# PASSIONLab/ELBA

Hardware: AMD Instinct MI355X
Metric: overlap nnz/sec (A·Aᵀ SpGEMM, SharedSeeds semiring, after Prune(numshared<=1)) (higher is better)
Workload: dtype u32

## Files before the change

### elba_amd/csrc/capi.hip

```cpp
#include "common.hpp"
#include "ov_plan.hpp"
#include <new>

using namespace elba;

struct elba_ctx {
    Ctx c;
};

namespace {

template <class F>
int guarded(elba_ctx *ctx, F &&f)
{
    if (!ctx) return ELBA_ERR_INVALID_ARG;
    try {
        ELBA_HIP(hipSetDevice(ctx->c.device));
        f(ctx->c);
        return ELBA_OK;
    } catch (const Error &e) {
        ctx->c.last_error = e.msg;
        return e.code;
    } catch (const std::bad_alloc &) {
        ctx->c.last_error = "host allocation failed";
// ... 753 lines not shown
        if (has(c.v, P_COUNTS)) { c.pre_ready = false; c.pre_consumed = true; }
    });
}

int elba_get_stat(elba_ctx *ctx, const char *name, int64_t *value)
{
    return guarded(ctx, [&](Ctx &c) {
        ELBA_REQUIRE(name && value, ELBA_ERR_INVALID_ARG, "get_stat: null name or value");
        if (!strcmp(name, "overlap_mirror_placed")) *value = c.ov_mir_placed;
        else if (!strcmp(name, "overlap_slab_q16")) *value = (int64_t)c.ov_slab_q16_used;
        else if (!strcmp(name, "kmer_path")) *value = c.kmer_path;
        else if (!strcmp(name, "kmer_passes")) *value = c.kmer_passes;
        else if (!strcmp(name, "kmer_crowded_buckets")) *value = c.kmer_crowded;
        else if (!strcmp(name, "kmer_crowded_small")) *value = c.kmer_crowded_small;
        else if (!strcmp(name, "kmer_largest_pass")) *value = c.kmer_largest_pass;
        else if (!strcmp(name, "kmer_peak_bytes")) *value = c.kmer_peak_bytes;
        else if (!strcmp(name, "kmer_buckets")) *value = c.kmer_buckets;
        else if (!strcmp(name, "overlap_passes")) *value = c.ov_passes;
        else if (!strcmp(name, "overlap_spec")) *value = c.ov_spec;
        else if (!strcmp(name, "overlap_forwarded")) *value = c.ov_forwarded;
        else if (!strncmp(name, "overlap_tier_limit_", 19) && name[19] >= '0' && name[19] < '0' + NUM_LDS_TIERS && !name[20]) *value = c.ov_tier_limit[name[19] - '0'];
        else if (!strncmp(name, "overlap_tier_queued_", 20) && name[20] >= '0' && name[20] < '0' + NUM_TIERS && !name[21]) *value = c.ov_tier_queued[name[20] - '0'];
        else if (!strncmp(name, "overlap_tier_done_", 18) && name[18] >= '0' && name[18] < '0' + NUM_TIERS && !name[19]) *value = c.ov_tier_done[name[18] - '0'];
        else if (!strcmp(name, "overlap_sort_rows_bucket")) *value = c.ov_sort_rows[0];
        else if (!strcmp(name, "overlap_sort_rows_huge")) *value = c.ov_sort_rows[1];
        else if (!strcmp(name, "overlap_family")) *value = c.ov_family;
        else if (!strcmp(name, "overlap_pay16")) *value = c.ov_pay16;
        else if (!strcmp(name, "overlap_rec16")) *value = c.ov_rec16_used;
        else if (!strcmp(name, "matrix_col_stride")) *value = has(c.v, P_A) && c.use_ell ? (int64_t)c.s_stride : 0;
        else if (!strcmp(name, "matrix_fbits")) *value = has(c.v, P_A) ? (int64_t)c.fbits : 0;
// ... 170 lines not shown
```

### elba_amd/csrc/common.hpp

```cpp
#pragma once
#include <hip/hip_runtime.h>
#include <cstdint>
#include <cstdio>
#include <cstdlib>
#include <cstring>
#include <mutex>
#include <string>
#include <vector>
#include "../../include/elba_amd.h"
#include "state.hpp"
#include "msd_plan.hpp"

namespace elba {

struct Error {
    int code;
    std::string msg;
};

#define ELBA_HIP(expr)                                                                                   \
    do {                                                                                                 \
        hipError_t e__ = (expr);                                                                         \
        if (e__ != hipSuccess) {                                                                         \
            throw ::elba::Error{e__ == hipErrorOutOfMemory ? ELBA_ERR_OUT_OF_MEMORY : ELBA_ERR_HIP,      \
// ... 159 lines not shown

    int64_t nreads = 0, first_global_id = 0, packed_bytes = 0;
    const uint8_t *d_packed = nullptr;
    const uint64_t *d_byte_off = nullptr;
    const uint32_t *d_len = nullptr;
    DevBuf own_packed, own_byte_off, own_len;
    uint32_t max_read_len = 0;
    std::vector<uint32_t> h_len;
    std::vector<uint64_t> h_byte_off;
    bool tx_index = false;
    DevBuf tx_recs, tx_name_pos, tx_name_len;
    std::vector<elba_fasta_record_t> tx_h_recs; std::vector<uint64_t> tx_h_name_pos; std::vector<uint32_t> tx_h_name_len;

    int triples_path = 0;
    int kmer_passes = 1;
    int64_t kmer_crowded = 0, kmer_crowded_small = 0, kmer_largest_pass = 0;
    int64_t kmer_peak_bytes = 0;
    int64_t kmer_buckets = 0;
    int kmer_path = 0;
    int64_t I = 0, ndistinct = 0;
    DevBuf inst_off;
    DevBuf rel_kmers;
    DevBuf rel_kmers_lo;
    DevBuf rel_kmers_lo2;
    DevBuf rel_counts;
    DevBuf csr_words;
    bool pre_pairs = false;
    bool pre_ready = false, pre_consumed = false, pre_words = false, pre_hints = false, pre_hints_done = false, pre_ell_done = false, pre_inline = false, pre_inline_pending = false ; int pre_rs = 0, pre_pbi = 0; int pre_nb = 0, pre_pb = 0; uint64_t pre_maxpos = 0;
    bool csr_hints = false, ov_hints_used = false, ov_rec16 = false;
    bool csr_inline = false;
// ... 215 lines not shown
```

### elba_amd/csrc/kmer.hip

```cpp
#include <memory>
#include "common.hpp"
#include "matrix.hpp"

namespace elba {

namespace {

#include "kmer_enum.hpp"

__device__ __forceinline__ uint64_t mix64(uint64_t k)
{
    k ^= k >> 33; k *= 0xff51afd7ed558ccdULL; k ^= k >> 33; k *= 0xc4ceb9fe1a85ec53ULL; k ^= k >> 33;
    return k;
}

__global__ void k_sort_columns(const uint32_t *colptr, uint64_t *csc, uint64_t *kid_keys, uint64_t N)
{
    const uint64_t k = (uint64_t)blockIdx.x * blockDim.x + threadIdx.x;
    if (k >= N) return;
    const uint32_t c0 = colptr[k], c1 = colptr[k + 1];
    for (uint32_t a = c0 + 1; a < c1; ++a) {
        const uint64_t v = csc[a];
        uint32_t b = a;
        while (b > c0 && csc[b - 1] > v) { csc[b] = csc[b - 1]; --b; }
// ... 485 lines not shown

    std::vector<uint64_t> off((size_t)M + 1);
    uint64_t I = 0;
    uint32_t maxlen = 0;
    for (int64_t r = 0; r < M; ++r) { const uint32_t l = c.h_len[(size_t)r]; off[(size_t)r] = I; if ((int64_t)l >= k) I += (uint64_t)l - k + 1; maxlen = l > maxlen ? l : maxlen; }
    off[(size_t)M] = I;
    c.max_read_len = maxlen;
    size_t free0 = 0;
    if (k > 31) { size_t total = 0; ELBA_HIP(hipMemGetInfo(&free0, &total)); }
    if (I >= 0xFFFFFFF0ull && k <= 31) {
        ELBA_REQUIRE(k >= 9, ELBA_ERR_UNSUPPORTED, "count_kmers: more than 2^32 k-mer instances on one GPU need k >= 9 (the sort of short k-mers holds 32-bit places)");
        ELBA_REQUIRE(!c.opt.kmer_no_msd, ELBA_ERR_UNSUPPORTED, "count_kmers: more than 2^32 k-mer instances on one GPU need the value partition (option kmer_no_msd is set)");
        ELBA_REQUIRE(k <= 17 || c.cfg.upper <= 255, ELBA_ERR_UNSUPPORTED, "count_kmers: more than 2^32 k-mer instances on one GPU need UPPER <= 255 for k > 17 (the sort holds 32-bit places)");
    }
    c.I = (int64_t)I; c.kmer_passes = 1; c.kmer_peak_bytes = 0;
    c.kmer_crowded = 0; c.kmer_crowded_small = 0; c.kmer_largest_pass = (int64_t)I; c.kmer_buckets = 0;
    c.inst_off.reserve((size_t)(M + 1) * 8);
    ELBA_HIP(hipMemcpyAsync(c.inst_off.p, off.data(), (size_t)(M + 1) * 8, hipMemcpyHostToDevice, s));

    if (k > 31) {
        const int words = k > 64 ? 3 : 2;
        if (count_long_kmers_in_passes(c, I, words, free0, st)) { done(c.v, EV_COUNT_KMERS); return; }
        DevBuf khi, klo, klo2, val, i0, i1, t0, t1, s2buf;
        for (DevBuf *b : {&khi, &klo, &val, &i0, &i1, &t0, &t1}) b->reserve((size_t)(I + 2) * 8);
        if (words == 3) { klo2.reserve((size_t)(I + 2) * 8); s2buf.reserve((size_t)(I + 2) * 8); }
        c.ws_a.reserve((size_t)(I + 2) * 8); c.ws_b.reserve((size_t)(I + 2) * 8); c.ws_c.reserve((size_t)(I + 2) * 8);
        c.ws_e.reserve((size_t)(I + 2) * 4); c.ws_f.reserve((size_t)(I + 2) * 8);
        c.t_total.start(s);
        c.t_a.start(s);
        EnumParams e = make_enum(c);
        const uint64_t nblocks = (I + EN_PER_BLOCK - 1) / EN_PER_BLOCK;
// ... 929 lines not shown
```

### elba_amd/csrc/kmer_msd.hip

```cpp
#include "common.hpp"
#include "matrix.hpp"
#include "msd_plan.hpp"
#include <algorithm>

namespace elba {

namespace {

#include "kmer_enum.hpp"

constexpr int MT_THREADS = ELBA_MT_THREADS, MT_ITEMS = ELBA_MT_ITEMS, MT_MAXBINS = 1 << MT_MAXBITS;
constexpr int BK_THREADS = 1024;
constexpr uint32_t EW = 2048;
constexpr uint32_t KW = EW / 2 + 1;
constexpr uint32_t EPAD = 256;
constexpr uint32_t BK_TAB = 16384, BK_ENT = BK_TAB + 2048 + 128 + 2 * (KW + 1);
static_assert(BK_ENT % 2 == 0, "staged entries are 8-byte words");
constexpr size_t BK_LDS_EMIT = (size_t)BK_ENT * 4 + (size_t)(EW + EPAD) * 10;
constexpr int KPT = 8;
static_assert(MT_ITEMS * 64 <= (1 << IB_SHIFT) && MT_TILE % 4096 == 0 && MT_TILE <= 65536, "a wavefront's share of a tile lies inside one block of the instance -> read table; run-start bitmap words per lane; 16-bit ranks");

struct MsdParams {
    int k2;
    int b1, b2;
// ... 206 lines not shown
            for (int u = 0; u < 8; ++u) x[u] = t + u < t1 ? hist[(size_t)(t + u) * nb2 + d] : 0u;
#pragma unroll
            for (int u = 0; u < 8; ++u) if (t + u < t1) hist[(size_t)(t + u) * nb2 + d] = x[u] + base;
        }
    }
    if (b == gridDim.x - 1 && d == 0) b2start[(size_t)gridDim.x * nb2] = (uint32_t)I;
}

#ifdef ELBA_SCATTER_CLOCK
__device__ unsigned long long g_sc_phase[2][2][12];
#define ELBA_SSTAMP(k) do { if (lane == 0 && w < 2) { const unsigned long long tn = __builtin_amdgcn_s_memtime(); sph[k] += tn - stp; stp = tn; } } while (0)
#else
#define ELBA_SSTAMP(k) do { } while (0)
#endif
__device__ __forceinline__ void lds_sync_fwd() { asm volatile("s_waitcnt lgkmcnt(0)\n\ts_barrier" ::: "memory"); }
template <bool ENUM, bool FILTER = false>
__global__ __launch_bounds__(MT_THREADS) void k_msd_scatter(EnumParams e, const BlockInfo *block_read, MsdParams m, const uint64_t *in, SegTiles sg, int shift, int bits,
                                                           const uint32_t *hist_scanned, uint64_t *out, uint32_t ntiles, uint32_t dlo, uint32_t dhi)
{
    __shared__ uint32_t kept_s;
    constexpr int WAVES = MT_THREADS / 64, DPT = MT_MAXBINS / MT_THREADS > 0 ? MT_MAXBINS / MT_THREADS : 1;
    __shared__ uint32_t lcnt[MT_MAXBINS], lstart[MT_MAXBINS], gbase[MT_MAXBINS], wsum[WAVES];
    __shared__ uint64_t lkey[MT_TILE];
    __shared__ unsigned long long hbits[MT_TILE / 64];
    __shared__ uint32_t hpre[MT_TILE / 64], delta[MT_MAXBINS];
    const uint32_t nbins = 1u << bits, dmask = nbins - 1u;
    if (!ENUM) ntiles = sg.tile0[sg.nb1];
    const int lane = threadIdx.x & 63, w = threadIdx.x >> 6;
    const unsigned long long lane_le = (2ull << lane) - 1ull;
#ifdef ELBA_SCATTER_CLOCK
    unsigned long long sph[12] = {0,0,0,0,0,0,0,0,0,0,0,0}, stp = __builtin_amdgcn_s_memtime();
#endif
    uint64_t key[MT_ITEMS];
    uint32_t dig2[MT_ITEMS / 2];
    uint32_t count = 0, ncount = 0; (void)ncount;
    auto digit = [&](int it) -> uint32_t { return (dig2[it >> 1] >> ((it & 1) * 16)) & 0xFFFFu; };
    auto set_digit = [&](int it, uint32_t d) { if (it & 1) dig2[it >> 1] |= d << 16; else dig2[it >> 1] = d; };
    auto fetch = [&](uint32_t t, uint32_t &cnt) {
        if (ENUM) {
            const uint64_t tbase = (uint64_t)t * MT_TILE, base = tbase + (uint64_t)w * (MT_ITEMS * 64);
            const uint64_t left = e.I - tbase;
            cnt = left < (uint64_t)MT_TILE ? (uint32_t)left : (uint32_t)MT_TILE;
            const uint64_t vmask = (1ull << (m.k2 - m.b1)) - 1;
#pragma unroll
            for (int it = 0; it < MT_ITEMS; ++it) key[it] = 0;
#pragma unroll
            for (int q = 0; q < MT_ITEMS / 2; ++q) dig2[q] = 0xFFFFFFFFu;
            enum_consecutive(e, block_read, base, [&](int it, uint64_t km, uint32_t r, uint32_t p) {
                const uint32_t dg = (uint32_t)(km >> (64 - m.b1));
                if (FILTER && (dg < dlo || dg >= dhi)) return;
                key[it] = (((km >> (64 - m.k2)) & vmask) << m.PB) | ((uint64_t)r << m.pbits) | p;
                dig2[it >> 1] = (it & 1) ? (dig2[it >> 1] & 0xFFFFu) | (dg << 16) : (dig2[it >> 1] & 0xFFFF0000u) | dg;
            });
        } else {
            uint32_t bucket, start;
            seg_tile(sg, t, bucket, start, cnt);
            const uint32_t wb = (uint32_t)w * (MT_ITEMS * 64);
#pragma unroll
            for (int it = 0; it < MT_ITEMS; ++it) {
                const uint32_t q = wb + (uint32_t)it * 64 + lane;
                key[it] = q < cnt ? in[start + q] : 0;
            }
        }
    };
    auto digits_of_loaded = [&](uint32_t cnt) {
        if (ENUM) return;
        const uint32_t wb = (uint32_t)w * (MT_ITEMS * 64);
#pragma unroll
        for (int it = 0; it < MT_ITEMS; ++it) {
            const uint32_t q = wb + (uint32_t)it * 64 + lane;
            set_digit(it, q < cnt ? (uint32_t)(key[it] >> shift) & dmask : 0xFFFFu);
        }
    };
#ifndef ELBA_SCATTER_ENUM_MODE
#define ELBA_SCATTER_ENUM_MODE 2
#endif
    constexpr bool PIPE = !ENUM || ELBA_SCATTER_ENUM_MODE != 0;
#ifndef ELBA_SCATTER_RR
    const uint32_t first_tile = (gridDim.x & 7u) ? blockIdx.x : (blockIdx.x & 7u) * (gridDim.x >> 3) + (blockIdx.x >> 3);
#else
    const uint32_t first_tile = blockIdx.x;
#endif
#ifndef ELBA_SCATTER_NO_PIPE
    if (PIPE && first_tile < ntiles) fetch(first_tile, count);
#endif
#ifndef ELBA_SCATTER_ONE_TILE
    for (uint32_t tile = first_tile; tile < ntiles; tile += gridDim.x) {
#else
    const uint32_t tile = blockIdx.x;
    if (tile < ntiles) {
#endif
    ELBA_SSTAMP(0);
// ... 21 lines not shown
    __syncthreads();
    ELBA_SSTAMP(3);
    {
        uint32_t tot[DPT], both = 0;
#pragma unroll
        for (int u = 0; u < DPT; ++u) { const uint32_t d = DPT * threadIdx.x + u; tot[u] = d < nbins ? lcnt[d] : 0u; both += tot[u]; }
        uint32_t inc = both;
#pragma unroll
        for (int s2 = 1; s2 < 64; s2 <<= 1) { const uint32_t o = __shfl_up(inc, s2, 64); if (lane >= s2) inc += o; }
        if (lane == 63) wsum[w] = inc;
        __syncthreads();
        uint32_t run = inc - both;
        for (int ww = 0; ww < w; ++ww) run += wsum[ww];
#pragma unroll
        for (int u = 0; u < DPT; ++u) { const uint32_t d = DPT * threadIdx.x + u; if (d < nbins) lstart[d] = run; run += tot[u]; }
        if (threadIdx.x == MT_THREADS - 1) kept_s = run;
#pragma unroll
        for (int u = 0; u < DPT; ++u) { const uint32_t d = threadIdx.x + u * MT_THREADS; if (d < nbins) gbase[d] = gb[u]; }
    }
    __syncthreads();
    ELBA_SSTAMP(4);
    if (ENUM && FILTER) count = kept_s;
#pragma unroll
    for (int it = 0; it < MT_ITEMS; ++it) {
        const uint32_t d = digit(it);
        if (d != 0xFFFFu) lkey[lstart[d] + rank[it]] = key[it];
    }
    ELBA_SSTAMP(5);
#ifdef ELBA_SCATTER_MEM_DIRECT
    if (!ENUM) {
#pragma unroll
        for (int u = 0; u < DPT; ++u) { const uint32_t d = DPT * threadIdx.x + u; if (d < nbins) delta[d] = gbase[d] - lstart[d]; }
        __syncthreads();
#pragma unroll
        for (int it = 0; it < MT_ITEMS; ++it) {
            const uint32_t t = (uint32_t)it * MT_THREADS + threadIdx.x;
            if (t < count) { const uint64_t kv = lkey[t]; out[delta[(uint32_t)(kv >> shift) & dmask] + t] = kv; }
        }
        __syncthreads();
#ifndef ELBA_SCATTER_ONE_TILE
        continue;
#else
        return;
#endif
    }
// ... 36 lines not shown
        const uint32_t t = (uint32_t)it * MT_THREADS + threadIdx.x;
        if (t < count) {
            const uint32_t run = hpre[t >> 6] + (uint32_t)__popcll(hbits[t >> 6] & ((2ull << (t & 63u)) - 1ull)) - 1u;
            out[delta[run] + t] = lkey[t];
        }
    }
#else
#if defined(ELBA_X_SCATTER) && ELBA_X_SCATTER == 1
    for (uint32_t t = threadIdx.x; t < count; t += MT_THREADS) out[(size_t)tile * MT_TILE + t] = lkey[t];
#elif defined(ELBA_X_SCATTER) && ELBA_X_SCATTER == 2
    for (uint32_t t = threadIdx.x; t < count; t += MT_THREADS) {
        const uint32_t run = hpre[t >> 6] + (uint32_t)__popcll(hbits[t >> 6] & lane_le) - 1u;
        if (delta[run] == 0xFFFFFFFEu) out[t] = lkey[t];
    }
#else
    if (ENUM) {
#pragma unroll 2
        for (uint32_t t = threadIdx.x; t < count; t += MT_THREADS) {
            const uint32_t run = hpre[t >> 6] + (uint32_t)__popcll(hbits[t >> 6] & lane_le) - 1u;
            out[delta[run] + t] = lkey[t];
        }
    } else
    for (uint32_t t = threadIdx.x; t < count; t += MT_THREADS) {
        const uint32_t run = hpre[t >> 6] + (uint32_t)__popcll(hbits[t >> 6] & lane_le) - 1u;
        out[delta[run] + t] = lkey[t];
    }
#endif
#endif
    };
#if !defined(ELBA_SCATTER_NO_PIPE) && !defined(ELBA_SCATTER_ONE_TILE)
    {
        const uint32_t nxt = tile + gridDim.x;
        const bool has = nxt < ntiles;
        if (!PIPE) writeout();
        else if (ENUM && ELBA_SCATTER_ENUM_MODE == 2 && (w & 1)) { writeout(); ELBA_SSTAMP(7); if (has) fetch(nxt, ncount); ELBA_SSTAMP(8); }
        else { if (has) fetch(nxt, ncount); ELBA_SSTAMP(8); writeout(); ELBA_SSTAMP(7); }
    }
#else
    writeout();
#endif
    lds_sync_fwd();
    ELBA_SSTAMP(9);
#ifndef ELBA_SCATTER_NO_PIPE
    if (PIPE) count = ncount;
#endif
    }
#ifdef ELBA_SCATTER_CLOCK
    if (lane == 0 && w < 2) for (int q = 0; q < 12; ++q) atomicAdd(&g_sc_phase[ENUM ? 1 : 0][w][q], sph[q]);
#endif
}

__device__ __forceinline__ void lds_sync() { asm volatile("s_waitcnt lgkmcnt(0)\n\ts_barrier" ::: "memory"); }

struct BucketStats { unsigned long long distinct, sumsq; unsigned int maxcol, ncrowded, nmid, nbig; };
struct BucketOut {
    uint64_t *rel_kmers; uint32_t *rel_counts, *colptr;
    uint64_t *csc, *csr_words, *kid_of_entry, *ell;
    uint32_t ell_stride;
    int nb, pb, rs, mb;
    uint32_t hints;
    uint32_t inl;
    unsigned long long *slot_cursor; uint32_t *slot_kid; uint32_t compact, slot_chunk;
    unsigned long long slot_cap;
    uint32_t *pair_key; uint64_t *pair_val;
// ... 1253 lines not shown

    void partition_triples()
    {
        const uint64_t I = pl.I;
        const uint32_t nb1 = pl.nb1, nb2 = pl.nb2, ntiles1 = pl.ntiles1, ntiles2 = pl.ntiles2;
        const SegTiles sg = seg();
        const uint32_t seg1[4] = {0u, (uint32_t)I, 0u, ntiles1};
        ELBA_HIP(hipMemcpyAsync(one_seg, seg1, sizeof(seg1), hipMemcpyHostToDevice, s));
        SegTiles sg1{one_seg, one_seg + 2, 1u};
        unsigned long long *badctr = reinterpret_cast<unsigned long long *>(one_seg + 4);
        ELBA_HIP(hipMemsetAsync(badctr, 0, 8, s));
        hipLaunchKernelGGL(k_pack_triple_msd, dim3((unsigned)((I + 255) / 256)), dim3(256), 0, s, tri->rows, tri->cols, tri->vals, I, tri->M, tri->N, m.pbits, m.PB, wb(), badctr);
        hipLaunchKernelGGL(k_msd_hist2, dim3(ntiles1), dim3(MT_THREADS), 0, s, (const uint64_t *)wb(), sg1, shift2() + m.b2, m.b1, hist());
        radix_column_scan(s, hist(), (int64_t)ntiles1, nb1, c.ws_scan);
        hipLaunchKernelGGL((k_tiles<MT_TILE, MT_MAXBINS>), dim3(1), dim3(MT_MAXBINS), 0, s, (const uint32_t *)hist(), nb1, I, b1start, tile0);
        hipLaunchKernelGGL((k_msd_scatter<false>), dim3(std::min<uint32_t>(ntiles1, sgrid())), dim3(MT_THREADS), 0, s, e, bi, m, (const uint64_t *)wb(), sg1, shift2() + m.b2, m.b1, (const uint32_t *)hist(), wa(), ntiles1, 0u, nb1);
        hipLaunchKernelGGL(k_msd_hist2, dim3(ntiles2), dim3(MT_THREADS), 0, s, (const uint64_t *)wa(), sg, shift2(), m.b2, hist());
        hipLaunchKernelGGL(k_msd_segscan, dim3(nb1), dim3(MT_MAXBINS), 0, s, hist(), sg, nb2, bt.b2start, I);
        hipLaunchKernelGGL((k_msd_scatter<false>), dim3(std::min<uint32_t>(ntiles2, sgrid())), dim3(MT_THREADS), 0, s, e, bi, m, (const uint64_t *)wa(), sg, shift2(), m.b2, (const uint32_t *)hist(), wb(), ntiles2, 0u, nb1);
        c.t_a.stop(s);
        c.t_b.start(s);
        ELBA_HIP(hipMemsetAsync(bt.gstat, 0, sizeof(BucketStats), s));
        hipLaunchKernelGGL(k_tri_stats, dim3((unsigned)std::min<uint32_t>(bt.nbuckets, (uint32_t)c.num_cus * 8u)), dim3(256), 0, s, (const uint64_t *)wb(), (const uint32_t *)bt.b2start, bt.nbuckets, m.PB, m.rkmask, pl.small_cap, bt.bN, bt.bZ, bt.gstat);
        bt.words = wb(); bt.wrel = wb();
        ps.on = false; sN = bt.bN; sZ = bt.bZ;
    }

    void partition_narrow(const Pass &pp, bool timed)
    {
        const uint32_t dlo = pp.dlo, dhi = pp.dhi, nb1 = pl.nb1, nb2 = pl.nb2, ntiles1 = pl.ntiles1, nbuckets = bt.nbuckets;
        const uint64_t Iv = pp.I;
        ELBA_REQUIRE(Iv + 2 <= std::min(c.ws_a.cap, c.ws_c.cap) / 8, ELBA_ERR_INTERNAL, "count_kmers: a value-range pass is larger than its partition buffers");
        const uint32_t nt2 = (uint32_t)((Iv + pl.tile - 1) / pl.tile) + nb1;
        const SegTiles sg = seg();
        if (timed) c.t_a.start(s);
        hipLaunchKernelGGL(k_msd_hist1, dim3(ntiles1), dim3(MT_THREADS), 0, s, e, bi, m, hist(), dlo, dhi);
        radix_column_scan(s, hist(), (int64_t)ntiles1, nb1, c.ws_scan);
        hipLaunchKernelGGL((k_tiles<MT_TILE, MT_MAXBINS>), dim3(1), dim3(MT_MAXBINS), 0, s, (const uint32_t *)hist(), nb1, Iv, b1start, tile0);
        if (pl.batched) hipLaunchKernelGGL((k_msd_scatter<true, true>), dim3(std::min<uint32_t>(ntiles1, sgrid())), dim3(MT_THREADS), 0, s, e, bi, m, (const uint64_t *)nullptr, sg, 0, m.b1, (const uint32_t *)hist(), wa(), ntiles1, dlo, dhi);
        else hipLaunchKernelGGL((k_msd_scatter<true, false>), dim3(std::min<uint32_t>(ntiles1, sgrid())), dim3(MT_THREADS), 0, s, e, bi, m, (const uint64_t *)nullptr, sg, 0, m.b1, (const uint32_t *)hist(), wa(), ntiles1, dlo, dhi);
        SegTiles sgi = sg; sgi.tinfo = tinfo;
        hipLaunchKernelGGL(k_msd_tile_info, dim3((nt2 + 255u) / 256u), dim3(256), 0, s, sg, tinfo);
        hipLaunchKernelGGL(k_msd_hist2, dim3(nt2), dim3(MT_THREADS), 0, s, (const uint64_t *)wa(), sgi, shift2(), m.b2, hist());
        hipLaunchKernelGGL(k_msd_segscan, dim3(nb1), dim3(MT_MAXBINS), 0, s, hist(), sg, nb2, bt.b2start, Iv);
        hipLaunchKernelGGL((k_msd_scatter<false>), dim3(std::min<uint32_t>(nt2, sgrid())), dim3(MT_THREADS), 0, s, e, bi, m, (const uint64_t *)wa(), sgi, shift2(), m.b2, (const uint32_t *)hist(), wb(), nt2, 0u, nb1);
#ifdef ELBA_SCATTER_CLOCK
        {
            ELBA_HIP(hipStreamSynchronize(s));
            unsigned long long h[2][2][12];
            ELBA_HIP(hipMemcpyFromSymbol(h, HIP_SYMBOL(g_sc_phase), sizeof(h)));
            static const char *nm[12] = {"top", "zero+bar", "rank", "bar", "scan+bar", "place", "bitmap+delta", "writeout", "fetch next", "end bar", "", ""};
            for (int en = 1; en >= 0; --en) for (int wv = 0; wv < 2; ++wv) {
                unsigned long long tot = 0; for (int q = 0; q < 12; ++q) tot += h[en][wv][q];
                fprintf(stderr, "k_msd_scatter<%s> wavefront %d:", en ? "ENUM" : "MEM", wv);
                for (int q = 0; q < 10; ++q) fprintf(stderr, " %s %.1f%%", nm[q], tot ? 100.0 * (double)h[en][wv][q] / (double)tot : 0.0);
                fprintf(stderr, "  (total %.0f cycles of the 100 MHz clock per workgroup)\n", (double)tot / 256.0);
            }
            unsigned long long z[2][2][12] = {};
            ELBA_HIP(hipMemcpyToSymbol(HIP_SYMBOL(g_sc_phase), z, sizeof(z)));
        }
#endif
        if (timed) { c.t_a.stop(s); c.t_b.start(s); }
        ELBA_HIP(hipMemsetAsync(bt.gstat, 0, sizeof(BucketStats), s));
        const unsigned bgrid = (unsigned)std::min<uint32_t>(nbuckets, (uint32_t)c.num_cus);
        if (m.rk != 0) hipLaunchKernelGGL(k_msd_count<true>, dim3(bgrid), dim3(BK_THREADS), CT_LDS, s, (const uint64_t *)wb(), (const uint32_t *)bt.b2start, nbuckets, m, pl.lower, pl.upper, pl.small_cap, bt.bN, bt.bZ, bt.gstat, bt.crowded, wa());
        else hipLaunchKernelGGL(k_msd_count<false>, dim3(bgrid), dim3(BK_THREADS), CT_LDS, s, (const uint64_t *)wb(), (const uint32_t *)bt.b2start, nbuckets, m, pl.lower, pl.upper, pl.small_cap, bt.bN, bt.bZ, bt.gstat, bt.crowded, wa());
        bt.words = wb(); bt.wrel = wa();
// ... 308 lines not shown
            ELBA_HIP(hipMemsetAsync(c.a_ell.as<char>() + (size_t)N * c.s_stride * 8, 0xFF, 64, s));
            emit_passes();
            ELBA_HIP(hipStreamSynchronize(s));
        } else if (compact) c.ell_nslots = (int64_t)slots[0];
        c.pre_ready = true; c.pre_consumed = false; c.pre_words = words; c.pre_hints = hints; c.pre_hints_done = hints && words; c.pre_ell_done = true; c.pre_inline_pending = false;
        c.pre_nb = nb; c.pre_pb = pb; c.pre_maxpos = pl.maxpos; c.pre_rs = rs; c.pre_inline = inl; c.pre_pbi = pbi;
        if (tri) return;
        elba_kmer_stats &st = *stp;
        st.instances = (int64_t)pl.I; st.distinct = (int64_t)hs.distinct; st.reliable = (int64_t)N; st.entries = (int64_t)Z;
        st.ms_total = c.t_total.ms(); st.ms_count = c.t_a.ms(); st.ms_sort = c.t_b.ms(); st.ms_lookup = 0;
        c.ndistinct = (int64_t)hs.distinct;
        c.N = (int64_t)N; c.Z = (int64_t)Z;
        c.kmer_path = pl.wide ? 2 : 1;
        c.kmer_passes = (int)passes.size();
        c.kmer_crowded = ncrowded; c.kmer_crowded_small = crowded_small; c.kmer_largest_pass = (int64_t)largest;
        c.kmer_buckets = 0;
        for (const Pass &pp : passes) c.kmer_buckets += (int64_t)pp.nb1 * pp.nb2;
    }
};

static bool msd_run(Ctx &c, uint64_t I, elba_kmer_stats *stp, MsdTriples *tri)
{
    if (c.opt.kmer_no_msd || c.opt.kmer_pairs || c.opt.kmer_unfused || c.opt.emit_plain || c.opt.kmer_drop) return false;
    if (tri && c.opt.csr_pairs) return false;
    MsdInput in{}; in.k = c.cfg.k; in.I = I; in.lower = (uint32_t)c.cfg.lower; in.upper = (uint32_t)c.cfg.upper;
    in.maxpos = tri ? tri->maxpos : reads_maxpos(c.max_read_len, c.cfg.k);
    in.nrows = tri ? tri->M : c.nreads; in.triN = tri ? tri->N : -1;
    MsdOptions op{}; op.kmer_msd = c.opt.kmer_msd; op.msd_wide_bits = c.opt.msd_wide_bits; op.msd_rank = c.opt.msd_rank; op.msd_no_rank = c.opt.msd_no_rank; op.msd_small_cap = c.opt.msd_small_cap; op.kmer_batch_instances = c.opt.kmer_batch_instances;
    const MsdPlan pl = plan_msd(in, op);
    if (!pl.ok) return false;
// ... 56 lines not shown
```

### elba_amd/csrc/msd_plan.hpp

```cpp
#pragma once
#include <algorithm>
#include <cstdint>
#include <vector>

#ifndef ELBA_MT_THREADS
#define ELBA_MT_THREADS 1024
#endif
#ifndef ELBA_MT_ITEMS
#define ELBA_MT_ITEMS 16
#endif
#ifndef ELBA_W2_THREADS
#define ELBA_W2_THREADS 512
#endif
#ifndef ELBA_W2_ITEMS
#define ELBA_W2_ITEMS 16
#endif

namespace elba {

constexpr int MT_TILE = ELBA_MT_THREADS * ELBA_MT_ITEMS;
constexpr int MT_MAXBITS = 9;
constexpr int VBITS = 16;
constexpr int W2_TILE = ELBA_W2_THREADS * ELBA_W2_ITEMS;
constexpr int W2_MAXBITS = 10;
constexpr uint32_t HINT_MAX_COL = 12;
constexpr uint32_t ES_CAP_MAX = 12288;
constexpr uint64_t MSD_PASS_LIMIT = 0xFFFFFFF0ull;

inline int bits_needed_u(uint64_t maxval)
{
    int b = 1;
    while (b < 64 && (maxval >> b)) ++b;
    return b;
}

// ... 4 lines not shown
inline uint64_t reads_maxpos(uint32_t max_read_len, int k) { return max_read_len >= (uint32_t)k ? max_read_len - (uint32_t)k : 0; }

struct MsdPlan {
    bool ok = false;
    bool tri = false, wide = false;
    bool batched = false;
    bool too_many_tiles = false;
    int k = 0, k2 = 0, T = 0, vb = VBITS;
    int b1 = 0, b2 = 0, pbits = 0, PB = 0, mb = 0, rk = 0;
    uint32_t rkmask = 0xFFFFFFFFu, dup = 0;
    uint32_t lower = 0, upper = 0;
    uint64_t I = 0, maxpos = 0, batch_cap = 0;
    int64_t nrows = 0;
    uint32_t nb1 = 0, nb2 = 0, nbuckets = 0;
    uint32_t tile = 0, ntiles1 = 0, ntiles2 = 0;
    uint32_t nb1_cap = 0, nbk_cap = 0;
    uint32_t small_cap = ES_CAP_MAX;
};

inline MsdPlan plan_msd(const MsdInput &in, const MsdOptions &opt)
{
    MsdPlan p{};
    const bool tri = in.triN >= 0;
    const int k = tri ? 17 : in.k, k2 = 2 * k;
    const uint64_t I = in.I;
    p.tri = tri; p.k = k; p.k2 = k2; p.I = I;
    if (k > 31 || (!tri && in.upper > 255) || I == 0) return p;
    const bool wide = !tri && k2 - VBITS > 2 * MT_MAXBITS;
    int T = k2 - VBITS, vb = VBITS;
    if (wide) {
// ... 21 lines not shown
    p.pbits = bits_needed_u(in.maxpos);
    p.mb = bits_needed_u((uint64_t)(in.nrows > 0 ? in.nrows - 1 : 0));
    p.PB = p.mb + p.pbits;
    if ((wide ? VBITS : tri ? T + vb : p.b2 + VBITS) + p.PB > 62) return p;
    p.rk = (p.PB + VBITS + 13 <= 64 && !opt.msd_no_rank && (wide || tri || p.upper > HINT_MAX_COL || opt.msd_rank)) ? p.PB + VBITS : 0;
    if (tri) { p.rk = p.PB; p.rkmask = (1u << vb) - 1u; p.dup = 1u; }
    p.nb1 = 1u << p.b1; p.nb2 = 1u << p.b2; p.nbuckets = p.nb1 * p.nb2;
    p.tile = wide ? (uint32_t)W2_TILE : (uint32_t)MT_TILE;
    p.batch_cap = opt.kmer_batch_instances > 0 ? (uint64_t)opt.kmer_batch_instances : 0xE0000000ull;
    p.batched = !tri && I > p.batch_cap;
    if (!p.batched && I >= MSD_PASS_LIMIT) return p;
    p.too_many_tiles = (I + p.tile - 1) / p.tile >= MSD_PASS_LIMIT;
    p.nb1_cap = wide && p.batched ? 1u << W2_MAXBITS : p.nb1;
    p.nbk_cap = wide && p.batched ? (1u << W2_MAXBITS) << W2_MAXBITS : p.nbuckets;
    p.ntiles1 = (uint32_t)((I + p.tile - 1) / p.tile); p.ntiles2 = p.ntiles1 + p.nb1_cap;
    p.small_cap = opt.msd_small_cap > 0 && (uint32_t)opt.msd_small_cap < ES_CAP_MAX ? (uint32_t)opt.msd_small_cap : ES_CAP_MAX;
    p.ok = true;
    return p;
}

struct Pass { uint32_t dlo = 0, dhi = 0; uint64_t I = 0, N = 0, Z = 0; uint32_t nb1 = 0, nb2 = 0; int T = 0, e = 0; int64_t ncrowded = 0, crowded_small = 0; uint32_t np = 0; };

inline Pass whole_pass(const MsdPlan &p) { Pass w{}; w.dlo = 0; w.dhi = p.nb1; w.I = p.I; w.nb1 = p.nb1; w.nb2 = p.nb2; w.T = p.T; return w; }

inline std::vector<Pass> plan_narrow_passes(const std::vector<unsigned long long> &dt, uint64_t batch_cap, uint32_t nb2, int T, int64_t *oversized = nullptr)
{
    const uint32_t nb1 = (uint32_t)dt.size();
    std::vector<Pass> passes;
    if (oversized) *oversized = -1;
    for (uint32_t d = 0; d < nb1;) {
// ... 35 lines not shown
```

Baseline: 16.92 billion.

## Add large-tile first-level MSD scatter kernel that stages packed reads in LDS

Replaces the enumerating variant of the first-level MSD scatter with a dedicated kernel. It uses much larger tiles, stores 16-bit local indices sorted by digit, and stages the tile's packed read bytes in shared memory so k-mers are re-extracted from LDS at writeout. A per-tile read table lets each k-mer's read and position be found by binary search. The aim is to cut repeated global reads and per-item enumeration cost in the k-mer counting partition step, at the price of more LDS use, lower occupancy and a slow fallback path. This runs in k-mer counting, not in the overlap SpGEMM being measured.

```diff
diff --git a/elba_amd/csrc/capi.hip b/elba_amd/csrc/capi.hip
--- a/elba_amd/csrc/capi.hip
+++ b/elba_amd/csrc/capi.hip
@@ -791,6 +791,7 @@
         else if (!strcmp(name, "kmer_crowded_buckets")) *value = c.kmer_crowded;
         else if (!strcmp(name, "kmer_crowded_small")) *value = c.kmer_crowded_small;
         else if (!strcmp(name, "kmer_largest_pass")) *value = c.kmer_largest_pass;
+        else if (!strcmp(name, "kmer_first_tile")) *value = c.kmer_first_tile;
         else if (!strcmp(name, "kmer_peak_bytes")) *value = c.kmer_peak_bytes;
         else if (!strcmp(name, "kmer_buckets")) *value = c.kmer_buckets;
         else if (!strcmp(name, "overlap_passes")) *value = c.ov_passes;
diff --git a/elba_amd/csrc/common.hpp b/elba_amd/csrc/common.hpp
--- a/elba_amd/csrc/common.hpp
+++ b/elba_amd/csrc/common.hpp
@@ -197,6 +197,7 @@
 
     int triples_path = 0;
     int kmer_passes = 1;
+    int64_t kmer_first_tile = 0;
     int64_t kmer_crowded = 0, kmer_crowded_small = 0, kmer_largest_pass = 0;
     int64_t kmer_peak_bytes = 0;
     int64_t kmer_buckets = 0;
diff --git a/elba_amd/csrc/kmer.hip b/elba_amd/csrc/kmer.hip
--- a/elba_amd/csrc/kmer.hip
+++ b/elba_amd/csrc/kmer.hip
@@ -523,7 +523,7 @@
         ELBA_REQUIRE(k <= 17 || c.cfg.upper <= 255, ELBA_ERR_UNSUPPORTED, "count_kmers: more than 2^32 k-mer instances on one GPU need UPPER <= 255 for k > 17 (the sort holds 32-bit places)");
     }
     c.I = (int64_t)I; c.kmer_passes = 1; c.kmer_peak_bytes = 0;
-    c.kmer_crowded = 0; c.kmer_crowded_small = 0; c.kmer_largest_pass = (int64_t)I; c.kmer_buckets = 0;
+    c.kmer_crowded = 0; c.kmer_crowded_small = 0; c.kmer_largest_pass = (int64_t)I; c.kmer_buckets = 0; c.kmer_first_tile = 0;
     c.inst_off.reserve((size_t)(M + 1) * 8);
     ELBA_HIP(hipMemcpyAsync(c.inst_off.p, off.data(), (size_t)(M + 1) * 8, hipMemcpyHostToDevice, s));
 
diff --git a/elba_amd/csrc/kmer_msd.hip b/elba_amd/csrc/kmer_msd.hip
--- a/elba_amd/csrc/kmer_msd.hip
+++ b/elba_amd/csrc/kmer_msd.hip
@@ -244,18 +244,16 @@
 #define ELBA_SSTAMP(k) do { } while (0)
 #endif
 __device__ __forceinline__ void lds_sync_fwd() { asm volatile("s_waitcnt lgkmcnt(0)\n\ts_barrier" ::: "memory"); }
-template <bool ENUM, bool FILTER = false>
 __global__ __launch_bounds__(MT_THREADS) void k_msd_scatter(EnumParams e, const BlockInfo *block_read, MsdParams m, const uint64_t *in, SegTiles sg, int shift, int bits,
                                                            const uint32_t *hist_scanned, uint64_t *out, uint32_t ntiles, uint32_t dlo, uint32_t dhi)
 {
-    __shared__ uint32_t kept_s;
     constexpr int WAVES = MT_THREADS / 64, DPT = MT_MAXBINS / MT_THREADS > 0 ? MT_MAXBINS / MT_THREADS : 1;
     __shared__ uint32_t lcnt[MT_MAXBINS], lstart[MT_MAXBINS], gbase[MT_MAXBINS], wsum[WAVES];
     __shared__ uint64_t lkey[MT_TILE];
     __shared__ unsigned long long hbits[MT_TILE / 64];
     __shared__ uint32_t hpre[MT_TILE / 64], delta[MT_MAXBINS];
     const uint32_t nbins = 1u << bits, dmask = nbins - 1u;
-    if (!ENUM) ntiles = sg.tile0[sg.nb1];
+    ntiles = sg.tile0[sg.nb1];
     const int lane = threadIdx.x & 63, w = threadIdx.x >> 6;
     const unsigned long long lane_le = (2ull << lane) - 1ull;
 #ifdef ELBA_SCATTER_CLOCK
@@ -267,34 +265,16 @@
     auto digit = [&](int it) -> uint32_t { return (dig2[it >> 1] >> ((it & 1) * 16)) & 0xFFFFu; };
     auto set_digit = [&](int it, uint32_t d) { if (it & 1) dig2[it >> 1] |= d << 16; else dig2[it >> 1] = d; };
     auto fetch = [&](uint32_t t, uint32_t &cnt) {
-        if (ENUM) {
-            const uint64_t tbase = (uint64_t)t * MT_TILE, base = tbase + (uint64_t)w * (MT_ITEMS * 64);
-            const uint64_t left = e.I - tbase;
-            cnt = left < (uint64_t)MT_TILE ? (uint32_t)left : (uint32_t)MT_TILE;
-            const uint64_t vmask = (1ull << (m.k2 - m.b1)) - 1;
-#pragma unroll
-            for (int it = 0; it < MT_ITEMS; ++it) key[it] = 0;
-#pragma unroll
-            for (int q = 0; q < MT_ITEMS / 2; ++q) dig2[q] = 0xFFFFFFFFu;
-            enum_consecutive(e, block_read, base, [&](int it, uint64_t km, uint32_t r, uint32_t p) {
-                const uint32_t dg = (uint32_t)(km >> (64 - m.b1));
-                if (FILTER && (dg < dlo || dg >= dhi)) return;
-                key[it] = (((km >> (64 - m.k2)) & vmask) << m.PB) | ((uint64_t)r << m.pbits) | p;
-                dig2[it >> 1] = (it & 1) ? (dig2[it >> 1] & 0xFFFFu) | (dg << 16) : (dig2[it >> 1] & 0xFFFF0000u) | dg;
-            });
-        } else {
-            uint32_t bucket, start;
-            seg_tile(sg, t, bucket, start, cnt);
-            const uint32_t wb = (uint32_t)w * (MT_ITEMS * 64);
-#pragma unroll
-            for (int it = 0; it < MT_ITEMS; ++it) {
-                const uint32_t q = wb + (uint32_t)it * 64 + lane;
-                key[it] = q < cnt ? in[start + q] : 0;
-            }
+        uint32_t bucket, start;
+        seg_tile(sg, t, bucket, start, cnt);
+        const uint32_t wb = (uint32_t)w * (MT_ITEMS * 64);
+#pragma unroll
+        for (int it = 0; it < MT_ITEMS; ++it) {
+            const uint32_t q = wb + (uint32_t)it * 64 + lane;
+            key[it] = q < cnt ? in[start + q] : 0;
         }
     };
     auto digits_of_loaded = [&](uint32_t cnt) {
-        if (ENUM) return;
         const uint32_t wb = (uint32_t)w * (MT_ITEMS * 64);
 #pragma unroll
         for (int it = 0; it < MT_ITEMS; ++it) {
@@ -302,10 +282,7 @@
             set_digit(it, q < cnt ? (uint32_t)(key[it] >> shift) & dmask : 0xFFFFu);
         }
     };
-#ifndef ELBA_SCATTER_ENUM_MODE
-#define ELBA_SCATTER_ENUM_MODE 2
-#endif
-    constexpr bool PIPE = !ENUM || ELBA_SCATTER_ENUM_MODE != 0;
+    constexpr bool PIPE = true;
 #ifndef ELBA_SCATTER_RR
     const uint32_t first_tile = (gridDim.x & 7u) ? blockIdx.x : (blockIdx.x & 7u) * (gridDim.x >> 3) + (blockIdx.x >> 3);
 #else
@@ -357,13 +334,11 @@
         for (int ww = 0; ww < w; ++ww) run += wsum[ww];
 #pragma unroll
         for (int u = 0; u < DPT; ++u) { const uint32_t d = DPT * threadIdx.x + u; if (d < nbins) lstart[d] = run; run += tot[u]; }
-        if (threadIdx.x == MT_THREADS - 1) kept_s = run;
 #pragma unroll
         for (int u = 0; u < DPT; ++u) { const uint32_t d = threadIdx.x + u * MT_THREADS; if (d < nbins) gbase[d] = gb[u]; }
     }
     __syncthreads();
     ELBA_SSTAMP(4);
-    if (ENUM && FILTER) count = kept_s;
 #pragma unroll
     for (int it = 0; it < MT_ITEMS; ++it) {
         const uint32_t d = digit(it);
@@ -371,7 +346,7 @@
     }
     ELBA_SSTAMP(5);
 #ifdef ELBA_SCATTER_MEM_DIRECT
-    if (!ENUM) {
+    {
 #pragma unroll
         for (int u = 0; u < DPT; ++u) { const uint32_t d = DPT * threadIdx.x + u; if (d < nbins) delta[d] = gbase[d] - lstart[d]; }
         __syncthreads();
@@ -438,13 +413,6 @@
         if (delta[run] == 0xFFFFFFFEu) out[t] = lkey[t];
     }
 #else
-    if (ENUM) {
-#pragma unroll 2
-        for (uint32_t t = threadIdx.x; t < count; t += MT_THREADS) {
-            const uint32_t run = hpre[t >> 6] + (uint32_t)__popcll(hbits[t >> 6] & lane_le) - 1u;
-            out[delta[run] + t] = lkey[t];
-        }
-    } else
     for (uint32_t t = threadIdx.x; t < count; t += MT_THREADS) {
         const uint32_t run = hpre[t >> 6] + (uint32_t)__popcll(hbits[t >> 6] & lane_le) - 1u;
         out[delta[run] + t] = lkey[t];
@@ -457,7 +425,6 @@
         const uint32_t nxt = tile + gridDim.x;
         const bool has = nxt < ntiles;
         if (!PIPE) writeout();
-        else if (ENUM && ELBA_SCATTER_ENUM_MODE == 2 && (w & 1)) { writeout(); ELBA_SSTAMP(7); if (has) fetch(nxt, ncount); ELBA_SSTAMP(8); }
         else { if (has) fetch(nxt, ncount); ELBA_SSTAMP(8); writeout(); ELBA_SSTAMP(7); }
     }
 #else
@@ -470,8 +437,173 @@
 #endif
     }
 #ifdef ELBA_SCATTER_CLOCK
-    if (lane == 0 && w < 2) for (int q = 0; q < 12; ++q) atomicAdd(&g_sc_phase[ENUM ? 1 : 0][w][q], sph[q]);
+    if (lane == 0 && w < 2) for (int q = 0; q < 12; ++q) atomicAdd(&g_sc_phase[0][w][q], sph[q]);
 #endif
+}
+
+constexpr int S1_THREADS = ELBA_MT1_THREADS, S1_ROUNDS = ELBA_MT1_ROUNDS, S1_WAVES = S1_THREADS / 64, S1_ITEMS = 16 * S1_ROUNDS;
+constexpr int S1_NBLK = MT_TILE1 >> IB_SHIFT;
+constexpr uint32_t S1_STAGE = MT_TILE1 / 4 + (MT_TILE1 > 32768 ? 4096 : 1024);
+constexpr uint32_t S1_WG_PER_CU = MT_TILE1 > 32768 ? 1u : 2u;
+constexpr uint32_t S1_RCAP = MT_TILE1 > 32768 ? 256u : 32u;
+static_assert(MT_TILE1 % MT_TILE == 0, "a first-level tile spans whole tiles of the first histogram");
+static_assert(S1_THREADS >= MT_MAXBINS && MT1_CHUNK <= (1 << IB_SHIFT) && MT_TILE1 % (1 << IB_SHIFT) == 0 && S1_STAGE % 8 == 0, "a thread per digit; a wavefront's chunk inside one table block; tiles start on a table block");
+__device__ __forceinline__ uint64_t twin64_brev(uint64_t w, int k)
+{
+    const uint64_t x = __builtin_bitreverse64(~w);
+    return (((x >> 1) & 0x5555555555555555ull) | ((x & 0x5555555555555555ull) << 1)) << (2 * (32 - k));
+}
+template <bool FILTER>
+__global__ __launch_bounds__(S1_THREADS, 4) void k_msd_scatter1(EnumParams e, const BlockInfo *block_read, MsdParams m, uint64_t packed_lim, const uint32_t *hist_scanned, uint64_t *out,
+                                                               uint32_t ntiles, uint32_t dlo, uint32_t dhi)
+{
+    __shared__ uint32_t lcnt[2][MT_MAXBINS], lstart[MT_MAXBINS], wsum[S1_WAVES], kept_s;
+    __shared__ uint16_t lidx[MT_TILE1];
+    __shared__ uint64_t lbase[S1_STAGE / 8];
+    __shared__ BlockInfo lblk[S1_NBLK + 1];
+    __shared__ uint32_t rst[S1_RCAP], lrd[S1_NBLK + 2], slow_s;
+    __shared__ uint2 rent[S1_RCAP];
+    constexpr int NST = (int)((S1_STAGE / 8 + S1_THREADS - 1) / S1_THREADS);
+    const uint32_t nbins = 1u << m.b1;
+    const uint32_t lane = threadIdx.x & 63, w = threadIdx.x >> 6;
+    const uint64_t nib = (e.I >> IB_SHIFT) + 1;
+    const uint64_t kmask = ~0ull << (64 - m.k2), vmask = (1ull << (m.k2 - m.b1)) - 1;
+    uint32_t dig2[S1_ITEMS / 2];
+    uint32_t count = 0, ncount = 0;
+    auto digit = [&](int it) -> uint32_t { return (dig2[it >> 1] >> ((it & 1) * 16)) & 0xFFFFu; };
+    auto fetch = [&](uint32_t t, uint32_t &cnt, uint32_t *cn) __attribute__((always_inline)) {
+        const uint64_t tbase = (uint64_t)t * MT_TILE1, left = e.I - tbase;
+        cnt = left < (uint64_t)MT_TILE1 ? (uint32_t)left : (uint32_t)MT_TILE1;
+#pragma unroll
+        for (int q = 0; q < S1_ITEMS / 2; ++q) dig2[q] = 0xFFFFFFFFu;
+        auto round = [&](auto qc) __attribute__((always_inline)) {
+            constexpr int q = decltype(qc)::value;
+            if constexpr (q < S1_ROUNDS)
+                enum_consecutive<16>(e, block_read, tbase + (uint64_t)((uint32_t)q * S1_WAVES + w) * MT1_CHUNK, [&](int it, uint64_t km, uint32_t, uint32_t) {
+                    const uint32_t dg = (uint32_t)(km >> (64 - m.b1));
+                    if (FILTER && (dg < dlo || dg >= dhi)) return;
+                    atomicAdd(&cn[dg], 1u);
+                    const int j = q * 16 + it;
+                    dig2[j >> 1] = (j & 1) ? (dig2[j >> 1] & 0xFFFFu) | (dg << 16) : (dig2[j >> 1] & 0xFFFF0000u) | dg;
+                });
+        };
+        static_assert(S1_ROUNDS <= 4, "rounds of a first-level tile");
+        round(std::integral_constant<int, 0>{}); round(std::integral_constant<int, 1>{}); round(std::integral_constant<int, 2>{}); round(std::integral_constant<int, 3>{});
+    };
+    const uint32_t first_tile = (gridDim.x & 7u) ? blockIdx.x : (blockIdx.x & 7u) * (gridDim.x >> 3) + (blockIdx.x >> 3);
+    if (threadIdx.x < MT_MAXBINS) lcnt[0][threadIdx.x] = 0;
+    __syncthreads();
+    if (first_tile < ntiles) fetch(first_tile, count, lcnt[0]);
+    __syncthreads();
+    uint32_t par = 0;
+    for (uint32_t tile = first_tile; tile < ntiles; tile += gridDim.x, par ^= 1u) {
+        const uint64_t tbase = (uint64_t)tile * MT_TILE1;
+        uint32_t *cur = lcnt[par], *nxc = lcnt[par ^ 1u];
+        if (threadIdx.x < MT_MAXBINS) nxc[threadIdx.x] = 0;
+        const BlockInfo b0 = block_read[tbase >> IB_SHIFT];
+        const uint64_t B0 = ((b0.byte_off != 0xFFFFFFFFu ? (uint64_t)b0.byte_off : e.byte_off[b0.read]) + (b0.pos0 >> 2)) & ~7ull;
+        uint64_t stg[NST];
+#pragma unroll
+        for (int u = 0; u < NST; ++u) {
+            const uint32_t i = (uint32_t)u * S1_THREADS + threadIdx.x;
+            const uint64_t a = B0 + (uint64_t)i * 8u;
+            stg[u] = (i < S1_STAGE / 8 && a + 8 <= packed_lim) ? *reinterpret_cast<const uint64_t *>(e.packed + a) : 0ull;
+        }
+        BlockInfo myblk = BlockInfo{e.nreads - 1u, 0u, 0u, 0xFFFFFFFFu};
+        if (threadIdx.x <= (uint32_t)S1_NBLK && (tbase >> IB_SHIFT) + threadIdx.x < nib) myblk = block_read[(tbase >> IB_SHIFT) + threadIdx.x];
+        const uint32_t gb = threadIdx.x < nbins ? hist_scanned[(size_t)tile * (MT_TILE1 / MT_TILE) * nbins + threadIdx.x] : 0u;
+        const uint32_t r_first = b0.read, r_last = (tbase >> IB_SHIFT) + S1_NBLK < nib ? block_read[(tbase >> IB_SHIFT) + S1_NBLK].read : e.nreads - 1u;
+        const bool rtab = r_last - r_first < S1_RCAP;
+        uint64_t my_ro = 0, my_ro1 = 0, my_bo = 0;
+        if (rtab && threadIdx.x <= r_last - r_first) { my_ro = e.inst_off[r_first + threadIdx.x]; my_ro1 = e.inst_off[r_first + threadIdx.x + 1u]; my_bo = e.byte_off[r_first + threadIdx.x]; }
+        if (threadIdx.x == 0) slow_s = rtab ? 0u : 1u;
+        {
+            const uint32_t tot = threadIdx.x < nbins ? cur[threadIdx.x] : 0u;
+            uint32_t inc = tot;
+#pragma unroll
+            for (int s2 = 1; s2 < 64; s2 <<= 1) { const uint32_t o = __shfl_up(inc, s2, 64); if (lane >= (uint32_t)s2) inc += o; }
+            if (lane == 63) wsum[w] = inc;
+            __syncthreads();
+            uint32_t run = inc - tot;
+            for (uint32_t ww = 0; ww < w; ++ww) run += wsum[ww];
+            if (threadIdx.x < nbins) { lstart[threadIdx.x] = run; cur[threadIdx.x] = gb - run; }
+            if (threadIdx.x == S1_THREADS - 1) kept_s = run + tot;
+        }
+        __syncthreads();
+        if (FILTER) count = kept_s;
+#pragma unroll
+        for (int it = 0; it < S1_ITEMS; ++it) {
+            const uint32_t d = digit(it);
+            if (d != 0xFFFFu) lidx[atomicAdd(&lstart[d], 1u)] = (uint16_t)(((uint32_t)(it >> 4) * S1_WAVES + w) * MT1_CHUNK + lane * 16u + (uint32_t)(it & 15));
+        }
+#pragma unroll
+        for (int u = 0; u < NST; ++u) { const uint32_t i = (uint32_t)u * S1_THREADS + threadIdx.x; if (i < S1_STAGE / 8) lbase[i] = __builtin_bswap64(stg[u]); }
+        if (threadIdx.x <= (uint32_t)S1_NBLK) lblk[threadIdx.x] = myblk;
+        if (rtab && threadIdx.x <= r_last - r_first) {
+            rst[threadIdx.x] = my_ro <= tbase ? 0u : (my_ro - tbase < (uint64_t)MT_TILE1 ? (uint32_t)(my_ro - tbase) : (uint32_t)MT_TILE1);
+            rent[threadIdx.x] = make_uint2((uint32_t)(tbase - my_ro), (uint32_t)(my_bo - B0));
+            const uint64_t tend = tbase + (e.I - tbase < (uint64_t)MT_TILE1 ? e.I - tbase : (uint64_t)MT_TILE1);
+            const uint64_t s0 = my_ro > tbase ? my_ro : tbase, s1 = my_ro1 < tend ? my_ro1 : tend;
+            if (s1 > s0) {
+                const uint64_t af = (my_bo + ((s0 - my_ro) >> 2)) & ~7ull, al = (my_bo + ((s1 - 1 - my_ro) >> 2)) & ~7ull;
+                if (af < B0 || al - B0 > (uint64_t)(S1_STAGE - 16u)) slow_s = 1u;
+            }
+        }
+        if (threadIdx.x <= (uint32_t)S1_NBLK) lrd[threadIdx.x] = myblk.read - r_first;
+        __syncthreads();
+        const bool fast = slow_s == 0u;
+        auto writeout = [&]() {
+            if (fast) {
+#pragma unroll 2
+                for (uint32_t t = threadIdx.x; t < count; t += S1_THREADS) {
+                    const uint32_t i = lidx[t];
+                    uint32_t lo = lrd[i >> IB_SHIFT], hi = lrd[(i >> IB_SHIFT) + 1u];
+                    while (hi - lo > 1u) { const uint32_t mid = (lo + hi) >> 1; if (rst[mid] <= i) lo = mid; else hi = mid - 1u; }
+                    const uint32_t j = rst[hi] <= i ? hi : lo;
+                    const uint2 en = rent[j];
+                    const uint32_t p = i + en.x, bb = en.y + (p >> 2), aw = bb >> 3, sh = (bb & 7u) * 8u + 2u * (p & 3u);
+                    const uint64_t w0 = lbase[aw], w1 = lbase[aw + 1u];
+                    const uint64_t fwd = (sh ? (w0 << sh) | (w1 >> (64u - sh)) : w0) & kmask, tw = twin64_brev(fwd, e.k), km = tw < fwd ? tw : fwd;
+                    const uint32_t d = (uint32_t)(km >> (64 - m.b1));
+                    out[cur[d] + t] = (((km >> (64 - m.k2)) & vmask) << m.PB) | ((uint64_t)(r_first + j) << m.pbits) | p;
+                }
+                return;
+            }
+#pragma unroll 2
+            for (uint32_t t = threadIdx.x; t < count; t += S1_THREADS) {
+                const uint32_t i = lidx[t], ib = i & ((1u << IB_SHIFT) - 1u);
+                const BlockInfo b = lblk[i >> IB_SHIFT];
+                uint32_t r = b.read, p = b.pos0 + ib;
+                uint64_t boff = b.byte_off;
+                if (ib >= b.remain) {
+                    const uint64_t g = tbase + i;
+                    uint32_t lo = b.read + 1u, hi = lblk[(i >> IB_SHIFT) + 1u].read;
+                    while (lo < hi) { const uint32_t mid = lo + ((hi - lo + 1u) >> 1); if (e.inst_off[mid] <= g) lo = mid; else hi = mid - 1u; }
+                    r = lo; p = (uint32_t)(g - e.inst_off[lo]); boff = e.byte_off[lo];
+                } else if (b.byte_off == 0xFFFFFFFFu) boff = e.byte_off[r];
+                const uint64_t bb = boff + (p >> 2), a = bb & ~7ull, rel = a - B0;
+                const uint32_t sh = (uint32_t)(bb - a) * 8u + 2u * (p & 3u);
+                uint64_t w0, w1;
+                if (rel <= (uint64_t)(S1_STAGE - 16u)) { w0 = lbase[rel >> 3]; w1 = lbase[(rel >> 3) + 1u]; }
+                else { const uint64_t *gw = reinterpret_cast<const uint64_t *>(e.packed + a); w0 = __builtin_bswap64(gw[0]); w1 = __builtin_bswap64(gw[1]); }
+                const uint64_t fwd = (sh ? (w0 << sh) | (w1 >> (64u - sh)) : w0) & kmask, tw = twin64(fwd, e.k), km = tw < fwd ? tw : fwd;
+                const uint32_t d = (uint32_t)(km >> (64 - m.b1));
+                out[cur[d] + t] = (((km >> (64 - m.k2)) & vmask) << m.PB) | ((uint64_t)r << m.pbits) | p;
+            }
+        };
+        {
+            const uint32_t nxt = tile + gridDim.x;
+            const bool has = nxt < ntiles;
+#if defined(ELBA_SCATTER_NO_PIPE)
+            writeout(); lds_sync_fwd(); if (has) fetch(nxt, ncount, nxc); lds_sync_fwd();
+#else
+            if (w & 1) { writeout(); if (has) fetch(nxt, ncount, nxc); }
+            else { if (has) fetch(nxt, ncount, nxc); writeout(); }
+            lds_sync_fwd();
+#endif
+        }
+        count = ncount;
+    }
 }
 
 __device__ __forceinline__ void lds_sync() { asm volatile("s_waitcnt lgkmcnt(0)\n\ts_barrier" ::: "memory"); }
@@ -1755,10 +1887,10 @@
         hipLaunchKernelGGL(k_msd_hist2, dim3(ntiles1), dim3(MT_THREADS), 0, s, (const uint64_t *)wb(), sg1, shift2() + m.b2, m.b1, hist());
         radix_column_scan(s, hist(), (int64_t)ntiles1, nb1, c.ws_scan);
         hipLaunchKernelGGL((k_tiles<MT_TILE, MT_MAXBINS>), dim3(1), dim3(MT_MAXBINS), 0, s, (const uint32_t *)hist(), nb1, I, b1start, tile0);
-        hipLaunchKernelGGL((k_msd_scatter<false>), dim3(std::min<uint32_t>(ntiles1, sgrid())), dim3(MT_THREADS), 0, s, e, bi, m, (const uint64_t *)wb(), sg1, shift2() + m.b2, m.b1, (const uint32_t *)hist(), wa(), ntiles1, 0u, nb1);
+        hipLaunchKernelGGL(k_msd_scatter, dim3(std::min<uint32_t>(ntiles1, sgrid())), dim3(MT_THREADS), 0, s, e, bi, m, (const uint64_t *)wb(), sg1, shift2() + m.b2, m.b1, (const uint32_t *)hist(), wa(), ntiles1, 0u, nb1);
         hipLaunchKernelGGL(k_msd_hist2, dim3(ntiles2), dim3(MT_THREADS), 0, s, (const uint64_t *)wa(), sg, shift2(), m.b2, hist());
         hipLaunchKernelGGL(k_msd_segscan, dim3(nb1), dim3(MT_MAXBINS), 0, s, hist(), sg, nb2, bt.b2start, I);
-        hipLaunchKernelGGL((k_msd_scatter<false>), dim3(std::min<uint32_t>(ntiles2, sgrid())), dim3(MT_THREADS), 0, s, e, bi, m, (const uint64_t *)wa(), sg, shift2(), m.b2, (const uint32_t *)hist(), wb(), ntiles2, 0u, nb1);
+        hipLaunchKernelGGL(k_msd_scatter, dim3(std::min<uint32_t>(ntiles2, sgrid())), dim3(MT_THREADS), 0, s, e, bi, m, (const uint64_t *)wa(), sg, shift2(), m.b2, (const uint32_t *)hist(), wb(), ntiles2, 0u, nb1);
         c.t_a.stop(s);
         c.t_b.start(s);
         ELBA_HIP(hipMemsetAsync(bt.gstat, 0, sizeof(BucketStats), s));
@@ -1769,29 +1901,31 @@
 
     void partition_narrow(const Pass &pp, bool timed)
     {
-        const uint32_t dlo = pp.dlo, dhi = pp.dhi, nb1 = pl.nb1, nb2 = pl.nb2, ntiles1 = pl.ntiles1, nbuckets = bt.nbuckets;
+        const uint32_t dlo = pp.dlo, dhi = pp.dhi, nb1 = pl.nb1, nb2 = pl.nb2, ntiles1 = pl.ntiles1, nt1 = pl.ntiles_first, nbuckets = bt.nbuckets;
         const uint64_t Iv = pp.I;
         ELBA_REQUIRE(Iv + 2 <= std::min(c.ws_a.cap, c.ws_c.cap) / 8, ELBA_ERR_INTERNAL, "count_kmers: a value-range pass is larger than its partition buffers");
         const uint32_t nt2 = (uint32_t)((Iv + pl.tile - 1) / pl.tile) + nb1;
         const SegTiles sg = seg();
         if (timed) c.t_a.start(s);
+        const uint64_t packed_lim = ((uint64_t)c.packed_bytes + 8u) & ~7ull;
+        const uint32_t grid1 = std::min<uint32_t>(nt1, (uint32_t)c.num_cus * S1_WG_PER_CU);
         hipLaunchKernelGGL(k_msd_hist1, dim3(ntiles1), dim3(MT_THREADS), 0, s, e, bi, m, hist(), dlo, dhi);
         radix_column_scan(s, hist(), (int64_t)ntiles1, nb1, c.ws_scan);
         hipLaunchKernelGGL((k_tiles<MT_TILE, MT_MAXBINS>), dim3(1), dim3(MT_MAXBINS), 0, s, (const uint32_t *)hist(), nb1, Iv, b1start, tile0);
-        if (pl.batched) hipLaunchKernelGGL((k_msd_scatter<true, true>), dim3(std::min<uint32_t>(ntiles1, sgrid())), dim3(MT_THREADS), 0, s, e, bi, m, (const uint64_t *)nullptr, sg, 0, m.b1, (const uint32_t *)hist(), wa(), ntiles1, dlo, dhi);
-        else hipLaunchKernelGGL((k_msd_scatter<true, false>), dim3(std::min<uint32_t>(ntiles1, sgrid())), dim3(MT_THREADS), 0, s, e, bi, m, (const uint64_t *)nullptr, sg, 0, m.b1, (const uint32_t *)hist(), wa(), ntiles1, dlo, dhi);
+        if (pl.batched) hipLaunchKernelGGL((k_msd_scatter1<true>), dim3(grid1), dim3(S1_THREADS), 0, s, e, bi, m, packed_lim, (const uint32_t *)hist(), wa(), nt1, dlo, dhi);
+        else hipLaunchKernelGGL((k_msd_scatter1<false>), dim3(grid1), dim3(S1_THREADS), 0, s, e, bi, m, packed_lim, (const uint32_t *)hist(), wa(), nt1, dlo, dhi);
         SegTiles sgi = sg; sgi.tinfo = tinfo;
         hipLaunchKernelGGL(k_msd_tile_info, dim3((nt2 + 255u) / 256u), dim3(256), 0, s, sg, tinfo);
         hipLaunchKernelGGL(k_msd_hist2, dim3(nt2), dim3(MT_THREADS), 0, s, (const uint64_t *)wa(), sgi, shift2(), m.b2, hist());
         hipLaunchKernelGGL(k_msd_segscan, dim3(nb1), dim3(MT_MAXBINS), 0, s, hist(), sg, nb2, bt.b2start, Iv);
-        hipLaunchKernelGGL((k_msd_scatter<false>), dim3(std::min<uint32_t>(nt2, sgrid())), dim3(MT_THREADS), 0, s, e, bi, m, (const uint64_t *)wa(), sgi, shift2(), m.b2, (const uint32_t *)hist(), wb(), nt2, 0u, nb1);
+        hipLaunchKernelGGL(k_msd_scatter, dim3(std::min<uint32_t>(nt2, sgrid())), dim3(MT_THREADS), 0, s, e, bi, m, (const uint64_t *)wa(), sgi, shift2(), m.b2, (const uint32_t *)hist(), wb(), nt2, 0u, nb1);
 #ifdef ELBA_SCATTER_CLOCK
         {
             ELBA_HIP(hipStreamSynchronize(s));
             unsigned long long h[2][2][12];
             ELBA_HIP(hipMemcpyFromSymbol(h, HIP_SYMBOL(g_sc_phase), sizeof(h)));
             static const char *nm[12] = {"top", "zero+bar", "rank", "bar", "scan+bar", "place", "bitmap+delta", "writeout", "fetch next", "end bar", "", ""};
-            for (int en = 1; en >= 0; --en) for (int wv = 0; wv < 2; ++wv) {
+            for (int en = 0; en >= 0; --en) for (int wv = 0; wv < 2; ++wv) {
                 unsigned long long tot = 0; for (int q = 0; q < 12; ++q) tot += h[en][wv][q];
                 fprintf(stderr, "k_msd_scatter<%s> wavefront %d:", en ? "ENUM" : "MEM", wv);
                 for (int q = 0; q < 10; ++q) fprintf(stderr, " %s %.1f%%", nm[q], tot ? 100.0 * (double)h[en][wv][q] / (double)tot : 0.0);
@@ -2130,6 +2264,7 @@
         c.kmer_path = pl.wide ? 2 : 1;
         c.kmer_passes = (int)passes.size();
         c.kmer_crowded = ncrowded; c.kmer_crowded_small = crowded_small; c.kmer_largest_pass = (int64_t)largest;
+        c.kmer_first_tile = (int64_t)pl.tile_first;
         c.kmer_buckets = 0;
         for (const Pass &pp : passes) c.kmer_buckets += (int64_t)pp.nb1 * pp.nb2;
     }
diff --git a/elba_amd/csrc/msd_plan.hpp b/elba_amd/csrc/msd_plan.hpp
--- a/elba_amd/csrc/msd_plan.hpp
+++ b/elba_amd/csrc/msd_plan.hpp
@@ -9,6 +9,15 @@
 #ifndef ELBA_MT_ITEMS
 #define ELBA_MT_ITEMS 16
 #endif
+#ifdef ELBA_MT1_TILE64K
+#define ELBA_MT1_THREADS 1024
+#endif
+#ifndef ELBA_MT1_THREADS
+#define ELBA_MT1_THREADS 512
+#endif
+#ifndef ELBA_MT1_ROUNDS
+#define ELBA_MT1_ROUNDS 4
+#endif
 #ifndef ELBA_W2_THREADS
 #define ELBA_W2_THREADS 512
 #endif
@@ -19,6 +28,9 @@
 namespace elba {
 
 constexpr int MT_TILE = ELBA_MT_THREADS * ELBA_MT_ITEMS;
+constexpr int MT1_CHUNK = 64 * 16;
+constexpr int MT_TILE1 = (ELBA_MT1_THREADS / 64) * ELBA_MT1_ROUNDS * MT1_CHUNK;
+static_assert(MT_TILE1 % MT1_CHUNK == 0 && MT_TILE1 <= 65536, "a place inside a first-level tile is a 16-bit index");
 constexpr int MT_MAXBITS = 9;
 constexpr int VBITS = 16;
 constexpr int W2_TILE = ELBA_W2_THREADS * ELBA_W2_ITEMS;
@@ -53,6 +65,7 @@
     int64_t nrows = 0;
     uint32_t nb1 = 0, nb2 = 0, nbuckets = 0;
     uint32_t tile = 0, ntiles1 = 0, ntiles2 = 0;
+    uint32_t tile_first = 0, ntiles_first = 0;
     uint32_t nb1_cap = 0, nbk_cap = 0;
     uint32_t small_cap = ES_CAP_MAX;
 };
@@ -104,6 +117,8 @@
     p.nb1_cap = wide && p.batched ? 1u << W2_MAXBITS : p.nb1;
     p.nbk_cap = wide && p.batched ? (1u << W2_MAXBITS) << W2_MAXBITS : p.nbuckets;
     p.ntiles1 = (uint32_t)((I + p.tile - 1) / p.tile); p.ntiles2 = p.ntiles1 + p.nb1_cap;
+    p.tile_first = wide || tri ? p.tile : (uint32_t)MT_TILE1;
+    p.ntiles_first = (uint32_t)((I + p.tile_first - 1) / p.tile_first);
     p.small_cap = opt.msd_small_cap > 0 && (uint32_t)opt.msd_small_cap < ES_CAP_MAX ? (uint32_t)opt.msd_small_cap : ES_CAP_MAX;
     p.ok = true;
     return p;
```

New measurement: 16.72 billion (median of 2 runs). Within noise of the previous version (-1.2%).
